# Karthik-Ragunath/RAD-NeRF

Measured on AMD Instinct MI355X. Metric: rendered frames/sec @512x512, higher is better.
Workload: dtype f32; 1 GPU; config[1]: inference 512x512, L=16 hash grid T=2^19 F=2 (xyz; ambient/torso grids tiled T=2^16 as shipped), max 16 steps/ray, 25 FPS pose stream, torso pass on; grid=hash19, engine=fused, frames_per_gpu=2122, table_dtype=f32, audio_batch=8, frames_in_flight=1, loop_launch=split, parallelism=frame-parallel x1

## Files before the change

include/radnerf_fused.h:

```cpp
#ifndef RADNERF_FUSED_H
#define RADNERF_FUSED_H

#include "radnerf_hip.h"

#ifdef __cplusplus
extern "C" {
#endif

typedef struct {
    const void *embeddings;
    const int32_t *offsets;
    uint32_t D, L, H;
    float S;
    uint32_t gridtype;
    int dtype;
} rn_grid_t;

typedef struct {
    const float *amb_w0, *amb_w1, *amb_w2;
    const float *sig_w0, *sig_w1, *sig_w2;
    const float *col_w0, *col_w1;
    uint32_t audio_dim, has_eye, ind_dim;
} rn_nerf_weights_t;

size_t rn_nerf_packed_floats(void);
size_t rn_nerf_packed_floats_h16(void);
int rn_nerf_pack_weights_h16(const rn_nerf_weights_t *w, float *packed, rn_stream_t stream);
#define RN_F32_SPLIT 2
size_t rn_nerf_packed_floats_split(void);
int rn_nerf_pack_weights_split(const rn_nerf_weights_t *w, float *packed, rn_stream_t stream);
size_t rn_nerf_bias_floats(void);
int rn_nerf_pack_weights(const rn_nerf_weights_t *w, float *packed, rn_stream_t stream);
int rn_nerf_frame_bias(const rn_nerf_weights_t *w, const float *enc_a, const float *eye, const float *ind_code,
                       float *bias, rn_stream_t stream);
int rn_nerf_frame_bias_batch(const rn_nerf_weights_t *w, const float *enc_a, uint32_t n, const float *eye, const float *ind_code,
                             float *bias, rn_stream_t stream);

int rn_nerf_fused_forward(const float *xyzs, const float *dirs, const float *deltas, uint32_t M,
                          const int32_t *m_dev, const rn_grid_t *grid_xyz, const rn_grid_t *grid_amb,
                          const float *packed, const float *bias, float bound, float *sigmas, float *rgbs,
                          float *ambient, int mlp_dtype, rn_stream_t stream);

#define RN_HEAD_STATE_INTS 64

typedef struct {
    const float *rays_o, *rays_d;
    uint32_t N;
    const float *aabb;
    float min_near;
    const uint8_t *bitfield;
    float bound, dt_gamma;
    uint32_t max_steps, cascade, grid_size;
    float T_thresh;
    float *nears, *fars;
    float *weights_sum, *depth, *image;
    int32_t *rays_alive_a, *rays_alive_b;
    float *rays_t;
    float *xyzs, *dirs, *deltas;
    float *sigmas, *rgbs;
    int32_t *state;
    uint32_t *block_counts;
    int32_t *live_slots;
    uint32_t order_w;
    const int32_t *occ_box;
} rn_head_t;

int rn_head_begin(const rn_head_t *h, rn_stream_t stream);
int rn_head_iterate(const rn_head_t *h, const rn_grid_t *grid_xyz, const rn_grid_t *grid_amb, const float *packed,
                    const float *bias, uint32_t first_iter, uint32_t n_iters, int mlp_dtype, rn_stream_t stream);
#define RN_LOOP_FIRST_MARCHED 1u
#define RN_LOOP_CLOSE_FRAME 2u
#define RN_LOOP_COOP 4u
int rn_head_iterate_ex(const rn_head_t *h, const rn_grid_t *grid_xyz, const rn_grid_t *grid_amb, const float *packed,
                       const float *bias, uint32_t first_iter, uint32_t n_iters, int mlp_dtype, uint32_t flags,
                       rn_stream_t stream);
int rn_frame_begin(const rn_head_t *h, const float *pose, float fx, float fy, float cx, float cy, uint32_t W,
                   rn_stream_t stream);
int rn_head_reschedule(const rn_head_t *h, uint32_t iter_done, uint32_t schedule_N, const int32_t *alive_total,
                       rn_stream_t stream);
#define RN_HEAD_ST_ACTIVE 4
#define RN_HEAD_ST_ITERS 16
#define RN_HEAD_ST_LIVE 17
#define RN_HEAD_ST_SLOTS 18
#define RN_HEAD_ST_UNFINISHED 19
#define RN_HEAD_ST_BARRIER 20
#define RN_HEAD_ST_STALLED 22
#define RN_HEAD_ST_HIST 32
int rn_head_check_done(const rn_head_t *h, uint32_t iters_done, rn_stream_t stream);

typedef struct {
    const float *def_w0, *def_w1, *def_w2;
    const float *tor_w0, *tor_w1, *tor_w2;
    uint32_t ind_dim;
} rn_torso_weights_t;
// ... 150 lines not shown
```

rad-nerf_amd/csrc/rn_grid.hip:

```cpp
#include "rn_scatter_dev.h"

#include <math.h>
#include <stdlib.h>

#ifndef RN_GRID_PAIR_HASHED
#define RN_GRID_PAIR_HASHED 1
#endif

namespace rn {

template <typename T, uint32_t D, uint32_t C, bool DYDX>
__device__ __forceinline__ void encode_one(const T *__restrict__ table, uint32_t off, const float (&in)[D], float scale,
                                           uint32_t resolution, uint32_t hashmap_size, uint32_t gridtype, bool align_corners,
                                           uint32_t interp, T (&results)[C], T (&grads)[DYDX ? D * C : 1]) {
    if constexpr (D == 2 || D == 3) {
        if (!align_corners && interp == 0) {
            const LevelPlan lp = plan_level<D>(scale, resolution, off, hashmap_size, gridtype, (uint32_t)(sizeof(T) * C));
            LevelFetch<T, D, C> f;
            issue_planned<T, D, C, RN_GRID_PAIR_HASHED != 0, true>(table, lp, in, f);
            blend_level<T, D, C, DYDX>(f, scale, results, grads);
            return;
        }
    }
    encode_level<T, D, C, DYDX>(table, off, in, scale, resolution, hashmap_size, gridtype, align_corners, interp, results, grads);
// ... 736 lines not shown
    if constexpr (C <= 2 && D <= 3)
        hipLaunchKernelGGL((k_grid_bwd_table_merge<T, D, C, LAYOUT>), grid, block, 0, a.stream, grad, a.inputs, a.offsets, gt, a.B, a.L,
                           a.lc, a.gridtype, a.align_corners, a.interp);
    else
        hipLaunchKernelGGL((k_grid_bwd_table<T, D, C, N_C, LAYOUT>), grid, block, 0, a.stream, grad, a.inputs, a.offsets, gt, a.B, a.L,
                           a.lc, a.gridtype, a.align_corners, a.interp);
    if (a.dy_dx && a.grad_inputs)
        hipLaunchKernelGGL((k_grid_bwd_input<T, D, C, LAYOUT>), dim3(div_up(a.B * D, 256)), block, 0, a.stream, grad,
                           static_cast<const T *>(a.dy_dx), static_cast<T *>(a.grad_inputs), a.B, a.L);
}
template <typename T, uint32_t D, uint32_t C>
static void launch_bwd(const BwdArgs &a) {
    if (a.layout == RN_LAYOUT_LBC) launch_bwd_layout<T, D, C, RN_LAYOUT_LBC>(a);
    else launch_bwd_layout<T, D, C, RN_LAYOUT_BLC>(a);
}
template <typename T, uint32_t D>
static int dispatch_bwd_c(uint32_t C, const BwdArgs &a) {
    switch (C) {
        case 1: launch_bwd<T, D, 1>(a); return RN_OK;
        case 2: launch_bwd<T, D, 2>(a); return RN_OK;
        case 4: launch_bwd<T, D, 4>(a); return RN_OK;
        case 8: launch_bwd<T, D, 8>(a); return RN_OK;
    }
    set_error("GridEncoding: C must be 1, 2, 4, or 8.");
    return RN_ERR_INVALID_ARG;
}
template <typename T>
static int dispatch_bwd_d(uint32_t D, uint32_t C, const BwdArgs &a) {
    switch (D) {
        case 2: return dispatch_bwd_c<T, 2>(C, a);
        case 3: return dispatch_bwd_c<T, 3>(C, a);
        case 4: return dispatch_bwd_c<T, 4>(C, a);
        case 5: return dispatch_bwd_c<T, 5>(C, a);
    }
    set_error("GridEncoding: D must be 2, 3, 4 or 5.");
    return RN_ERR_INVALID_ARG;
}

template <uint32_t D>
static int dispatch_tv_c(uint32_t C, const float *inputs, const float *table, float *grad, const int32_t *offsets,
                         float weight, uint32_t B, uint32_t L, const LevelConsts &lc, uint32_t gridtype, bool ac,
                         hipStream_t s) {
    const dim3 block(256), grid(div_up(B, 256), L);
    switch (C) {
        case 1: hipLaunchKernelGGL((k_grad_tv<D, 1>), grid, block, 0, s, inputs, table, grad, offsets, weight, B, lc, gridtype, ac); return RN_OK;
        case 2: hipLaunchKernelGGL((k_grad_tv<D, 2>), grid, block, 0, s, inputs, table, grad, offsets, weight, B, lc, gridtype, ac); return RN_OK;
        case 4: hipLaunchKernelGGL((k_grad_tv<D, 4>), grid, block, 0, s, inputs, table, grad, offsets, weight, B, lc, gridtype, ac); return RN_OK;
        case 8: hipLaunchKernelGGL((k_grad_tv<D, 8>), grid, block, 0, s, inputs, table, grad, offsets, weight, B, lc, gridtype, ac); return RN_OK;
    }
    set_error("GridEncoding: C must be 1, 2, 4, or 8.");
    return RN_ERR_INVALID_ARG;
}

}

using namespace rn;

extern "C" {

int rn_grid_encode_forward(const float *inputs, const void *embeddings, const int32_t *offsets, void *outputs,
                           uint32_t B, uint32_t D, uint32_t C, uint32_t L, float S, uint32_t H, void *dy_dx,
                           uint32_t gridtype, int align_corners, uint32_t interp, int dtype, int layout,
                           rn_stream_t stream) {
    if (B == 0) return RN_OK;
    RN_REQUIRE(inputs && embeddings && offsets && outputs, "grid_encode_forward: null pointer");
    RN_REQUIRE(L >= 1 && L <= kMaxLevels, "grid_encode_forward: L=%u out of range (1..%u)", L, kMaxLevels);
    RN_REQUIRE(dtype == RN_F32 || dtype == RN_F16, "grid_encode_forward: dtype must be RN_F32 or RN_F16");
    RN_REQUIRE(layout == RN_LAYOUT_LBC || layout == RN_LAYOUT_BLC || layout == RN_LAYOUT_BLC_LEVELMAJOR,
               "grid_encode_forward: bad layout");
    RN_REQUIRE(gridtype <= 1 && interp <= 1, "grid_encode_forward: bad gridtype / interpolation id");
    FwdArgs a{inputs, embeddings, offsets, outputs, B, L, make_level_consts(L, S, H), dy_dx, gridtype,
              align_corners != 0, interp, layout, as_stream(stream)};
    const int rc = (dtype == RN_F32) ? dispatch_fwd_d<float>(D, C, a) : dispatch_fwd_d<__half>(D, C, a);
    if (rc != RN_OK) return rc;
    return check_launch("grid_encode_forward");
}

size_t rn_grid_encode_forward_workspace(uint32_t B, uint32_t L, uint32_t C, int dtype) {
    const size_t per_sample = (size_t)L * C * (dtype == RN_F16 ? 2 : 4);
    const size_t chunk = B < planned_chunk_default() ? B : planned_chunk_default();
    return chunk * per_sample;
}

static int grid_forward_ws(const float *inputs, const void *embeddings, const int32_t *offsets, const int32_t *offsets_host,
                           void *outputs, uint32_t B, uint32_t D, uint32_t C, uint32_t L, float S, uint32_t H, void *dy_dx,
                           uint32_t gridtype, int align_corners, uint32_t interp, int dtype, int layout, void *workspace,
                           size_t workspace_bytes, const InXform &xf, rn_stream_t stream, const char *who) {
    if (B == 0) return RN_OK;
    RN_REQUIRE(inputs && embeddings && offsets && outputs, "%s: null pointer", who);
    RN_REQUIRE(L >= 1 && L <= kMaxLevels, "%s: L=%u out of range (1..%u)", who, L, kMaxLevels);
    RN_REQUIRE(dtype == RN_F32 || dtype == RN_F16, "%s: dtype must be RN_F32 or RN_F16", who);
    RN_REQUIRE(layout == RN_LAYOUT_LBC || layout == RN_LAYOUT_BLC, "%s: layout must be RN_LAYOUT_LBC or RN_LAYOUT_BLC", who);
    const bool shape_ok = offsets_host && !dy_dx && !align_corners && interp == 0 && (D == 2 || D == 3) && (C == 2 || C == 4) &&
                          ((uintptr_t)embeddings & 15u) == 0 && ((uintptr_t)outputs & 15u) == 0 &&
                          (layout == RN_LAYOUT_LBC || (workspace && ((uintptr_t)workspace & 15u) == 0));
    if (shape_ok) {
        PlannedArgs a{inputs, embeddings, offsets, offsets_host, outputs, B, L, make_level_consts(L, S, H), gridtype, layout, workspace,
                      workspace_bytes, as_stream(stream), xf};
        const int rc = (dtype == RN_F32) ? dispatch_planned<float>(D, C, a) : dispatch_planned<__half>(D, C, a);
        if (rc <= 0) return rc != RN_OK ? rc : check_launch(who);
    }
    RN_REQUIRE(!xf.on, "%s: only the planned shapes (offsets_host given, D in {2,3}, C in {2,4}, 16-byte aligned buffers); normalise the "
               "coordinates yourself and call rn_grid_encode_forward_ws", who);
    return rn_grid_encode_forward(inputs, embeddings, offsets, outputs, B, D, C, L, S, H, dy_dx, gridtype, align_corners, interp, dtype,
                                  layout, stream);
}

int rn_grid_encode_forward_ws(const float *inputs, const void *embeddings, const int32_t *offsets, const int32_t *offsets_host,
                              void *outputs, uint32_t B, uint32_t D, uint32_t C, uint32_t L, float S, uint32_t H, void *dy_dx,
                              uint32_t gridtype, int align_corners, uint32_t interp, int dtype, int layout, void *workspace,
                              size_t workspace_bytes, rn_stream_t stream) {
// ... 55 lines not shown
```

rad-nerf_amd/radnerf/fused.py:

```python
import ctypes as C

import numpy as np
import torch

import radnerf_hip as hip
from radnerf_hip.abi import (RN_F16, RN_F32, RN_F32_SPLIT, RN_HEAD_ST_HIST, RN_HEAD_ST_ITERS, RN_HEAD_ST_SLOTS, RN_HEAD_ST_STALLED,
                             RN_HEAD_ST_UNFINISHED, RN_HEAD_STATE_INTS, RN_LOOP_CLOSE_FRAME, RN_LOOP_COOP, RN_LOOP_FIRST_MARCHED,
                             RN_TORSO_PLAN_MAX_BYTES, GridT, HeadT, NerfWeightsT, TorsoWeightsT)

from . import switches

_lib = hip._lib


def _grid_desc(enc, table):
    g = GridT()
    g.embeddings, g.offsets = table.data_ptr(), enc.offsets.data_ptr()
    g.D, g.L, g.H = enc.input_dim, enc.num_levels, enc.base_resolution
    g.S = float(np.log2(enc.per_level_scale))
    g.gridtype = enc.gridtype_id
    g.dtype = RN_F16 if table.dtype == torch.float16 else RN_F32
    return g


def head_weights(model):
    return [l.weight for l in model.ambient_net.net] + [l.weight for l in model.sigma_net.net] + [l.weight for l in model.color_net.net]


def weights_desc(ws, audio_dim, has_eye, ind_dim):
    nw = NerfWeightsT()
    (nw.amb_w0, nw.amb_w1, nw.amb_w2, nw.sig_w0, nw.sig_w1, nw.sig_w2, nw.col_w0, nw.col_w1) = [w.data_ptr() for w in ws]
    nw.audio_dim, nw.has_eye, nw.ind_dim = audio_dim, has_eye, ind_dim
    return nw


def torso_weights(model):
    return [l.weight for l in model.torso_deform_net.net] + [l.weight for l in model.torso_net.net]


def torso_weights_desc(ws, ind_dim):
    assert tuple(ws[0].shape) == (64, 96 + ind_dim) and tuple(ws[3].shape) == (32, 128 + ind_dim)
    tw = TorsoWeightsT()
    (tw.def_w0, tw.def_w1, tw.def_w2, tw.tor_w0, tw.tor_w1, tw.tor_w2) = [w.data_ptr() for w in ws]
    tw.ind_dim = ind_dim
    return tw


def torso_constants(poses, ind_code):
    return (poses.detach().reshape(-1).contiguous().float(),
            ind_code.detach().reshape(-1).contiguous().float() if ind_code is not None else None)


def supported(model):
    try:
        ok = (model.encoder.num_levels == 16 and model.encoder.level_dim == 2 and model.encoder.input_dim == 3
              and model.encoder_ambient.num_levels == 16 and model.encoder_ambient.level_dim == 2
              and model.encoder_ambient.input_dim == 2 and model.hidden_dim == 64 and model.geo_feat_dim == 64
              and model.hidden_dim_ambient == 64 and model.hidden_dim_color == 64 and model.num_layers == 3
              and model.num_layers_ambient == 3 and model.num_layers_color == 2 and model.ambient_dim == 2
              and model.encoder_dir.degree == 4 and not model.encoder.align_corners and model.encoder.interp_id == 0)
        if model.torso:
            ok = ok and (model.torso_encoder.num_levels == 16 and model.torso_encoder.level_dim == 2
                         and model.torso_deform_net.dim_hidden == 64 and model.torso_net.dim_hidden == 32
                         and model.torso_deform_in_dim == 42 and model.pose_in_dim == 54)
        return bool(ok)
    except AttributeError:
        return False


class TorsoPlan:

    def __init__(self, key, refs, buf, n_on, stream):
        self.key, self.refs, self.buf, self.n_on, self.stream = key, refs, buf, n_on, stream
        self.event = torch.cuda.Event()
        self.event.record()
        self.waited = {stream}


class FusedState:

    def __init__(self, model):
        if not supported(model):
            raise RuntimeError("fused engine: unsupported network shape; use engine='ops'")
        self.model = model
        self.dev = model.density_bitfield.device
        n_packed = max(int(_lib.rn_nerf_packed_floats()), int(_lib.rn_nerf_packed_floats_h16()),
                       int(_lib.rn_nerf_packed_floats_split()))
        self.packed = torch.empty(n_packed, dtype=torch.float32, device=self.dev)
        self.mlp_dtype = RN_F32
        self.loop_hint = None
        self.bias = torch.empty(int(_lib.rn_nerf_bias_floats()), dtype=torch.float32, device=self.dev)
        self.tpacked = (torch.empty(int(_lib.rn_torso_packed_floats()), dtype=torch.float32, device=self.dev)
                        if model.torso else None)
        self._versions = None
        self._N = 0
        self._zero_eye = torch.zeros(1, dtype=torch.float32, device=self.dev)
        self.plan = None
        self.plan_builds = 0
        self.box = None
        self._box_key = None
        self.box_builds = 0

    def occ_box(self):
        if not switches.on("RN_OCC_BOX"):
            return None
        m = self.model
        bits = m.density_bitfield
        key = (bits.data_ptr(), bits._version, int(m.cascade), int(m.grid_size))
        if key != self._box_key:
            if self.box is None:
                self.box = torch.zeros(8, dtype=torch.int32, device=self.dev)
            hip.call("rn_occ_box", hip.ptr(bits), int(m.cascade), int(m.grid_size), hip.ptr(self.box), hip.stream())
            self._box_key = key
            self.box_builds += 1
        return self.box

    def _weights(self):
        m = self.model
        ws = head_weights(m)
        if m.torso:
            ws += torso_weights(m)
        return ws

    def refresh(self):
        ws = self._weights()
        tables = [self.model.encoder.embeddings, self.model.encoder_ambient.embeddings]
        if self.model.torso:
            tables.append(self.model.torso_encoder.embeddings)
        mlp = {"f32": RN_F32, "f16": RN_F16, "f32x2": RN_F32_SPLIT}[
            getattr(getattr(self.model, "opt", None), "mlp_dtype", "f32")]
        half = bool(getattr(getattr(self.model, "opt", None), "half_tables", False))
        versions = tuple((w._version, w.data_ptr()) for w in ws + tables) + (mlp, half)
        if versions == self._versions:
            return
        m = self.model
        for w in ws:
            if w.dtype != torch.float32 or not w.is_contiguous():
                raise RuntimeError("fused engine: MLP weights must be contiguous float32")
        self.nw = weights_desc(ws[:8], m.audio_dim, int(m.exp_eye), m.individual_dim)
        assert tuple(ws[0].shape) == (64, 32 + m.audio_dim) and tuple(ws[3].shape) == (64, 64 + int(m.exp_eye))
        assert tuple(ws[5].shape) == (65, 64) and tuple(ws[6].shape) == (64, 80 + m.individual_dim)
        self.mlp_dtype = mlp
        packer = {RN_F32: "rn_nerf_pack_weights", RN_F16: "rn_nerf_pack_weights_h16",
                  RN_F32_SPLIT: "rn_nerf_pack_weights_split"}[mlp]
        hip.call(packer, C.byref(self.nw), hip.ptr(self.packed), hip.stream())
        if m.torso:
            self.tw = torso_weights_desc(ws[8:14], m.individual_dim_torso)
            hip.call("rn_torso_pack_weights", C.byref(self.tw), hip.ptr(self.tpacked), hip.stream())
        if half:
            encs = [m.encoder, m.encoder_ambient] + ([m.torso_encoder] if m.torso else [])
            self.tables = [hip.aligned(e.half_table()) for e in encs]
        else:
            self.tables = [hip.aligned(t.detach()) for t in tables]
        self.gx = _grid_desc(m.encoder, self.tables[0])
# ... 237 lines not shown
        alpha_out = torch.empty(N, 1, dtype=torch.float32, device=dev)
    hip.call("rn_torso_fused", hip.ptr(bg_coords), N, hip.ptr(model.density_grid_torso), int(model.grid_size), float(thresh),
             hip.ptr(poses6), hip.ptr(ict), float(model.opt.torso_shrink), C.byref(st.tw), hip.ptr(st.tpacked), C.byref(st.gt),
             hip.ptr(bg_in), hip.ptr(bg_out), hip.ptr(alpha_out), hip.ptr(deform_out), hip.stream())
    return bg_out, alpha_out


def frame_bias_batch(model, codes, eye, ind_code):
    st = _state(model)
    st.refresh()
    return _frame_bias(st, codes, eye, ind_code, batch=True)


def render_frame(model, rays_o, rays_d, enc_a, ind_code, eye, bg_coords, poses, ind_code_torso, bg_color, dt_gamma,
                 max_steps, T_thresh, want_u8=False, ray_source=None, frame_bias=None):
    st = _state(model)
    st.refresh()
    N = rays_o.shape[0]
    st.scratch(N)
    dev = rays_o.device
    s = hip.stream()

    if frame_bias is None:
        bias = _frame_bias(st, enc_a, eye, ind_code)
    else:
        bias = frame_bias.reshape(-1)
        assert bias.numel() == st.bias.numel() and bias.is_contiguous() and bias.dtype == torch.float32

    weights_sum = torch.empty(N, dtype=torch.float32, device=dev)
    depth = torch.empty(N, dtype=torch.float32, device=dev)
    image = torch.empty(N, 3, dtype=torch.float32, device=dev)

    h = HeadT()
    h.rays_o, h.rays_d, h.N = rays_o.data_ptr(), rays_d.data_ptr(), N
    h.aabb, h.min_near = model.aabb_infer.data_ptr(), float(model.min_near)
    h.bitfield, h.bound, h.dt_gamma = model.density_bitfield.data_ptr(), float(model.bound), float(dt_gamma)
    h.max_steps, h.cascade, h.grid_size, h.T_thresh = int(max_steps), int(model.cascade), int(model.grid_size), float(T_thresh)
    h.nears, h.fars = st.nears.data_ptr(), st.fars.data_ptr()
    h.weights_sum, h.depth, h.image = weights_sum.data_ptr(), depth.data_ptr(), image.data_ptr()
    h.rays_alive_a, h.rays_alive_b = st.rays_alive[0].data_ptr(), st.rays_alive[1].data_ptr()
    h.rays_t = st.rays_t.data_ptr()
    h.xyzs = st.samples.data_ptr()
    h.dirs = st.samples.data_ptr() + N * 3 * 4
    h.deltas = st.samples.data_ptr() + N * 6 * 4
    h.sigmas, h.rgbs = st.sigmas.data_ptr(), st.rgbs.data_ptr()
    h.state, h.block_counts = st.state.data_ptr(), st.block_counts.data_ptr()
    h.live_slots = st.live_slots.data_ptr() if (getattr(model.opt, "live_list", True) and switches.on("RN_LIVE_LIST")) else None
    h.order_w = int(getattr(model, "ray_order_width", 0) or 0)
    h.occ_box = hip.ptr(st.occ_box())

    shard = getattr(model, "shard_schedule", None)
    merged = shard is None and getattr(model.opt, "frame_kernels", "merged") == "merged"
    n_iters = int(max_steps) if st.loop_hint is None else min(int(max_steps), st.loop_hint)
    if merged:
        if ray_source is not None:
            pose, (fx, fy, cx, cy), W = ray_source
            pose = pose.reshape(-1, 4)[:4].contiguous().float()
            hip.call("rn_frame_begin", C.byref(h), hip.ptr(pose), float(fx), float(fy), float(cx), float(cy), int(W), s)
        else:
            hip.call("rn_frame_begin", C.byref(h), None, 0.0, 0.0, 0.0, 0.0, 0, s)
        hip.call("rn_head_iterate_ex", C.byref(h), C.byref(st.gx), C.byref(st.gw), hip.ptr(st.packed), hip.ptr(bias), 0, n_iters,
                 st.mlp_dtype, RN_LOOP_FIRST_MARCHED | RN_LOOP_CLOSE_FRAME | loop_flags(model), s)
    else:
        if ray_source is not None:
            pose, (fx, fy, cx, cy), W = ray_source
            pose = pose.reshape(-1, 4)[:4].contiguous().float()
            hip.call("rn_get_rays", hip.ptr(pose), float(fx), float(fy), float(cx), float(cy), N // int(W), int(W), hip.ptr(rays_o),
                     hip.ptr(rays_d), s)
        hip.call("rn_head_begin", C.byref(h), s)
        if shard is None:
            hip.call("rn_head_iterate_ex", C.byref(h), C.byref(st.gx), C.byref(st.gw), hip.ptr(st.packed), hip.ptr(bias), 0,
                     n_iters, st.mlp_dtype, loop_flags(model), s)
        else:
            group, n_total = shard
            total = torch.empty(1, dtype=torch.int32, device=dev)
            for it in range(n_iters):
                hip.call("rn_head_iterate_ex", C.byref(h), C.byref(st.gx), C.byref(st.gw), hip.ptr(st.packed), hip.ptr(bias),
                         it, 1, st.mlp_dtype, loop_flags(model), s)
                bank = ((it + 1) & 1) * 8
                total.copy_(st.state[bank:bank + 1])
                group.all_reduce(total)
                hip.call("rn_head_reschedule", C.byref(h), it, int(n_total), hip.ptr(total), hip.stream())
        if n_iters < int(max_steps):
            hip.call("rn_head_check_done", C.byref(h), n_iters, s)

    bg_in = None
    if torch.is_tensor(bg_color):
        bg_in = bg_color.reshape(-1, 3).contiguous().float()
        if bg_in.shape[0] != N:
            bg_in = bg_in.expand(N, 3).contiguous()
    elif bg_color is not None and float(bg_color) != 1.0:
        bg_in = torch.full((N, 3), float(bg_color), dtype=torch.float32, device=dev)
    results = {}
    model.last_stats = LoopStats(st)
    u8 = torch.empty(N, 3, dtype=torch.uint8, device=dev) if want_u8 else None
    if model.torso and merged:
        thresh = min(model.density_thresh_torso, model.mean_density_torso)
        keep = getattr(model.opt, "keep_torso_layer", True)
        talpha = torch.empty(N, 1, dtype=torch.float32, device=dev) if keep else None
        bg_final = torch.empty(N, 3, dtype=torch.float32, device=dev) if keep else None
        coords = bg_coords.contiguous().float()
        p6, ict = torso_constants(poses, ind_code_torso)
        plan = st.torso_plan(bg_coords, coords, thresh)
        if plan is not None:
            hip.call("rn_torso_blend_frame_planned", hip.ptr(plan.buf), plan.buf.numel(), N, plan.n_on, hip.ptr(p6), hip.ptr(ict),
                     float(model.opt.torso_shrink), C.byref(st.tw), hip.ptr(st.tpacked), C.byref(st.gt), hip.ptr(bg_in),
                     hip.ptr(bg_final), hip.ptr(talpha), None, hip.ptr(image), hip.ptr(weights_sum), hip.ptr(depth),
                     hip.ptr(st.nears), hip.ptr(st.fars), hip.ptr(u8), s)
        else:
            hip.call("rn_torso_blend_frame", hip.ptr(coords), N, hip.ptr(model.density_grid_torso), int(model.grid_size), float(thresh),
                     hip.ptr(p6), hip.ptr(ict), float(model.opt.torso_shrink), C.byref(st.tw), hip.ptr(st.tpacked), C.byref(st.gt),
                     hip.ptr(bg_in), hip.ptr(bg_final), hip.ptr(talpha), hip.ptr(image), hip.ptr(weights_sum), hip.ptr(depth),
                     hip.ptr(st.nears), hip.ptr(st.fars), hip.ptr(u8), s)
        if keep:
            results["torso_alpha"], results["torso_color"] = talpha, bg_final
    else:
        bg_final = bg_in
        if model.torso:
            thresh = min(model.density_thresh_torso, model.mean_density_torso)
            bg_final, talpha = torso_forward(model, bg_coords, poses, ind_code_torso, thresh, bg_in=bg_in)
            results["torso_alpha"], results["torso_color"] = talpha, bg_final
        hip.call("rn_blend_frame", hip.ptr(image), hip.ptr(weights_sum), hip.ptr(bg_final), hip.ptr(depth), hip.ptr(st.nears),
                 hip.ptr(st.fars), N, hip.ptr(u8), s)
    results.update(image=image, depth=depth, weights_sum=weights_sum, nears=st.nears, fars=st.fars)
    if want_u8:
        results["image_u8"] = u8
    return results


def get_rays(pose, intrinsics, H, W):
# ... 20 lines not shown
```

rad-nerf_amd/radnerf/switches.py:

```python
import os

TABLE = (
    ("RN_ADAM", "hip", ("hip", "torch"), "optimizer of `make_optimizer` on the GPU: `HipAdam` (one update kernel for all tensors) or torch's fused Adam"),
    ("RN_ASR", "torch", ("torch", "hip"), "`Wav2Vec2CTC` (`radnerf/asr.py`) on the GPU in fp32: the same arithmetic in plain torch, or the wav2vec2 kernels (`rn_asr_*`, opt-in: bit-reproducible and independent of the batching, but 56 ms against 44 ms for a minute of audio at the real size, DESIGN.md §3)"),
    ("RN_AUDIO_TRAIN", "hip", ("hip", "torch"), "`encode_audio` on the GPU: the audio kernels (`radnerf/audio.py`) or the `nn.Module` path"),
    ("RN_LIVE_LIST", "1", ("1", "0"), "fused inference engine: hand the loop the list of live sample slots (`0`: every launch scans all slots)"),
    ("RN_MLP_TRAIN", "hip", ("hip", "torch"), "the per-operator MLP stacks under autograd: `rn_mlp64_*` (`radnerf/mlp_train.py`) or `nn.Linear`"),
    ("RN_OCC_BOX", "1", ("1", "0"), "fused inference engine: hand the loop the box around the occupancy grid's set bits (`rn_occ_box`, built once per grid): with one cascade and a constant step a ray tests only the cells between its entry into and its exit from that box (same bits); `0`: every ray tests every cell from `near` to `far`"),
    ("RN_PERCEP", "hip", ("hip", "torch"), "`PerceptualAlex` (`radnerf/percep.py`) on the GPU in fp32: the perceptual kernels (`rn_percep_*`), or the same arithmetic in plain torch (unfold + matmul)"),
    ("RN_SCATTER", "lbc", ("lbc", "binned"), "table-gradient scatter: the line merge for every level, or hashed levels of the first grid summed by table region"),
    ("RN_TORSO_PLAN", "1", ("1", "0"), "fused inference engine: a frame whose pixel grid and torso occupancy grid are those of the frame before runs its torso pass over a plan built once (`rn_torso_plan_build`: the covered pixels and their position encoding; same bits); `0`: every frame computes them (`rn_torso_blend_frame`)"),
    ("RN_TORSO_STEP", "device", ("device", "host"), "with `RN_TORSO_TRAIN=fused`: the whole torso step on a device-side count, or the fused layer on the index list the host asks for"),
    ("RN_TORSO_TRAIN", "ops", ("ops", "fused"), "torso layer of a training call: the per-operator layers, or the fused kernels of `radnerf/train_torso.py` (opt-in)"),
    ("RN_TRAIN_CAMERA", "torch", ("torch", "fused"), "pose code of `--train_camera`: torch's expressions, or `rn_camera_rays_*` (`radnerf/train_camera.py`, opt-in; lets a captured camera step keep the fused head)"),
    ("RN_TRAIN_DETERMINISTIC", "0", ("0", "1"), "`1`: a step on the fused routes (head, `RN_TRAIN_CAMERA=fused`, `RN_TORSO_TRAIN=fused`) runs no float atomic, eager or captured: the table gradients are summed in one fixed order (`rn_grid_scatter_ordered`; takes precedence over `RN_SCATTER`) and the audio nets' parameter gradients through per-workgroup partials -- two runs from the same seeds give the same bits (opt-in: slower)"),
    ("RN_TRAIN_GLUE", "hip", ("hip", "torch"), "elementwise glue of the per-operator step: single kernels (`radnerf/train_glue.py`) or the PyTorch expressions"),
    ("RN_TRAIN_HEAD", "fused", ("fused", "ops"), "`NeRFNetwork.forward` of a training call: one forward and one backward kernel (`radnerf/train_head.py`) or the per-operator path"),
    ("RN_TRAIN_HEAD_ZERO", "0", ("0", "1"), "`1`: the fused head zero-fills its output rows past the live count (for tools that look at all rows)"),
    ("RN_TRAIN_LOSS", "fused", ("fused", "torch"), "head loss of `train_step`: blend, clamp and loss in one kernel, or the PyTorch expression"),
    ("RN_TRAIN_MARCH", "step", ("step", "ops"), "marcher of a budgeted step: one launch with near / far and the counters, or `near_far_from_aabb` + `rn_march_rays_train_budget`"),
    ("RN_TRAIN_MLP", "f32", ("f32", "f16"), "matrix products of the fused head (`RN_TRAIN_HEAD=fused`): fp32 matrix cores, or 16-bit operands with fp32 sums (`rn_train_head_*_h16`, opt-in: the arithmetic of the reference's `-O` runs for its `nn.Linear` layers; saved tiles, tables and gradients stay fp32)"),
    ("RN_TRAIN_NOISE", "hash", ("hash", "torch"), "jitter of the one-launch marcher: the launch's own hash, or `torch.rand` as the reference draws it (the test suite pins this)"),
    ("RN_TRAIN_OVERLAP", "1", ("1", "0"), "table-gradient scatter and audio nets on side streams beside the step (`0`: everything on one stream)"),
    ("RN_TRAIN_PACKED", "1", ("1", "0"), "`SyntheticTrainStream.batch`: one gather kernel into one flat buffer (`0`: separate tensors, as a generic loader hands over)"),
    ("RN_TRAIN_SET", "hip", ("hip", "torch"), "`DeviceTrainSet.batch` on the GPU: one launch, or the plain-torch restatement of `collate`"),
)
_ROWS = {row[0]: row for row in TABLE}


def get(name):
    _, default, accepted, _ = _ROWS[name]
    value = os.environ.get(name, default)
    if value not in accepted:
        raise ValueError(f"{name}={value!r} is not one of its accepted values: {' | '.join(accepted)}")
    return value


def on(name):
    return get(name) == "1"


def markdown():
    rows = ["| switch | default | accepted | selects |", "|---|---|---|---|"]
    rows += ["| `%s` | `%s` | %s | %s |" % (name, default, " \\| ".join("`%s`" % v for v in accepted), doc) for name, default, accepted, doc in TABLE]
    return "\n".join(rows)


if __name__ == "__main__":
    print(markdown())
```

rad-nerf_amd/radnerf_hip/abi.py:

```python
import ctypes as C

_int, _u32, _f32, _f64, _sz, _ptr, _P = C.c_int, C.c_uint32, C.c_float, C.c_double, C.c_size_t, C.c_void_p, C.POINTER
_i64 = C.c_int64

RN_F32, RN_F16 = 0, 1
RN_LAYOUT_LBC, RN_LAYOUT_BLC, RN_LAYOUT_BLC_LEVELMAJOR = 0, 1, 2

RN_F32_SPLIT = 2
RN_HEAD_STATE_INTS = 64
RN_TORSO_PLAN_MAX_BYTES = 256 << 20
RN_LOOP_FIRST_MARCHED, RN_LOOP_CLOSE_FRAME, RN_LOOP_COOP = 1, 2, 4
RN_HEAD_ST_ACTIVE, RN_HEAD_ST_ITERS, RN_HEAD_ST_LIVE, RN_HEAD_ST_SLOTS = 4, 16, 17, 18
RN_HEAD_ST_UNFINISHED, RN_HEAD_ST_STALLED, RN_HEAD_ST_HIST = 19, 22, 32


class GridT(C.Structure):
    c_name = "rn_grid_t"
    _fields_ = [("embeddings", _ptr), ("offsets", _ptr), ("D", _u32), ("L", _u32), ("H", _u32), ("S", _f32),
                ("gridtype", _u32), ("dtype", _int)]


class NerfWeightsT(C.Structure):
    c_name = "rn_nerf_weights_t"
    _fields_ = [("amb_w0", _ptr), ("amb_w1", _ptr), ("amb_w2", _ptr), ("sig_w0", _ptr), ("sig_w1", _ptr),
# ... 77 lines not shown
    "rn_device_count": (_int, []),
    "rn_prof_enable": (_int, [_int]),
    "rn_prof_pause": (_int, [_int]),
    "rn_prof_collect": (_int, [C.POINTER(_u32), C.POINTER(_f32)]),
    "rn_prof_durations": (_int, [C.POINTER(_f32), _u32]),
    "rn_near_far_from_aabb": (_int, [_ptr, _ptr, _ptr, _u32, _f32, _ptr, _ptr, _ptr]),
    "rn_sph_from_ray": (_int, [_ptr, _ptr, _f32, _u32, _ptr, _ptr]),
    "rn_morton3D": (_int, [_ptr, _u32, _ptr, _ptr]),
    "rn_morton3D_invert": (_int, [_ptr, _u32, _ptr, _ptr]),
    "rn_packbits": (_int, [_ptr, _u32, _f32, _ptr, _ptr]),
    "rn_morton3D_dilation": (_int, [_ptr, _u32, _u32, _ptr, _ptr]),
    "rn_march_rays_train_workspace": (_sz, [_u32]),
    "rn_march_rays_train": (_int, [_ptr, _ptr, _ptr, _f32, _f32, _u32, _u32, _u32, _u32, _u32, _ptr, _ptr, _ptr, _ptr, _ptr,
                                   _ptr, _ptr, _ptr, _ptr, _ptr]),
    "rn_march_rays_train_budget": (_int, [_ptr, _ptr, _ptr, _f32, _f32, _u32, _u32, _u32, _u32, _u32, _ptr, _ptr, _ptr, _ptr,
                                          _ptr, _ptr, _ptr, _ptr, _ptr, _ptr, _ptr]),
    "rn_march_rays_train_step_state": (_sz, [_u32]),
    "rn_march_rays_train_step": (_int, [_ptr, _ptr, _ptr, _ptr, _f32, _f32, _f32, _u32, _u32, _u32, _u32, _u32, _ptr, _ptr,
                                        _ptr, _ptr, _ptr, _ptr, _ptr, _ptr, _ptr, _ptr, _u32, _ptr]),
    "rn_march_rays_train_backward": (_int, [_ptr, _ptr, _ptr, _ptr, _u32, _u32, _ptr, _ptr, _ptr]),
    "rn_composite_rays_train_forward": (_int, [_ptr, _ptr, _ptr, _ptr, _ptr, _u32, _u32, _f32, _ptr, _ptr, _ptr, _ptr, _ptr]),
    "rn_composite_rays_train_backward": (_int, [_ptr, _ptr, _ptr, _ptr, _ptr, _ptr, _ptr, _ptr, _ptr, _ptr, _ptr, _u32, _u32,
                                                _f32, _ptr, _ptr, _ptr, _ptr]),
    "rn_march_rays": (_int, [_u32, _u32, _ptr, _ptr, _ptr, _ptr, _f32, _f32, _u32, _u32, _u32, _ptr, _ptr, _ptr, _ptr, _ptr,
                             _ptr, _ptr, _ptr, _ptr]),
    "rn_composite_rays": (_int, [_u32, _u32, _f32, _ptr, _ptr, _ptr, _ptr, _ptr, _ptr, _ptr, _ptr, _ptr, _ptr]),
    "rn_compact_rays_workspace": (_sz, [_u32]),
    "rn_compact_rays": (_int, [_ptr, _u32, _ptr, _ptr, _ptr, _ptr, _ptr]),
    "rn_grid_encode_forward": (_int, [_ptr, _ptr, _ptr, _ptr, _u32, _u32, _u32, _u32, _f32, _u32, _ptr, _u32, _int, _u32, _int,
                                      _int, _ptr]),
    "rn_grid_encode_forward_workspace": (_sz, [_u32, _u32, _u32, _int]),
    "rn_grid_encode_forward_ws": (_int, [_ptr, _ptr, _ptr, _ptr, _ptr, _u32, _u32, _u32, _u32, _f32, _u32, _ptr, _u32, _int,
                                         _u32, _int, _int, _ptr, _sz, _ptr]),
    "rn_grid_encode_forward_bound": (_int, [_ptr, _f32, _ptr, _ptr, _ptr, _ptr, _u32, _u32, _u32, _u32, _f32, _u32, _u32, _int,
                                            _int, _ptr, _sz, _ptr]),
    "rn_grid_encode_backward": (_int, [_ptr, _ptr, _ptr, _ptr, _ptr, _u32, _u32, _u32, _u32, _f32, _u32, _ptr, _ptr, _u32, _int,
                                       _u32, _int, _int, _ptr]),
    "rn_grad_total_variation": (_int, [_ptr, _ptr, _ptr, _ptr, _f32, _u32, _u32, _u32, _u32, _f32, _u32, _u32, _int, _ptr]),
    "rn_sh_encode_forward": (_int, [_ptr, _ptr, _u32, _u32, _u32, _ptr, _ptr]),
    "rn_sh_encode_backward": (_int, [_ptr, _ptr, _u32, _u32, _u32, _ptr, _ptr, _ptr]),
    "rn_freq_encode_forward": (_int, [_ptr, _u32, _u32, _u32, _u32, _ptr, _ptr]),
    "rn_freq_encode_backward": (_int, [_ptr, _ptr, _u32, _u32, _u32, _u32, _ptr, _ptr]),
    "rn_nerf_packed_floats": (_sz, []),
    "rn_nerf_packed_floats_h16": (_sz, []),
    "rn_nerf_pack_weights_h16": (_int, [_P(NerfWeightsT), _ptr, _ptr]),
    "rn_nerf_packed_floats_split": (_sz, []),
    "rn_nerf_pack_weights_split": (_int, [_P(NerfWeightsT), _ptr, _ptr]),
    "rn_nerf_bias_floats": (_sz, []),
    "rn_nerf_pack_weights": (_int, [_P(NerfWeightsT), _ptr, _ptr]),
    "rn_nerf_frame_bias": (_int, [_P(NerfWeightsT), _ptr, _ptr, _ptr, _ptr, _ptr]),
    "rn_nerf_frame_bias_batch": (_int, [_P(NerfWeightsT), _ptr, _u32, _ptr, _ptr, _ptr, _ptr]),
    "rn_nerf_fused_forward": (_int, [_ptr, _ptr, _ptr, _u32, _ptr, _P(GridT), _P(GridT), _ptr, _ptr, _f32, _ptr, _ptr, _ptr,
                                     _int, _ptr]),
    "rn_head_begin": (_int, [_P(HeadT), _ptr]),
    "rn_head_iterate": (_int, [_P(HeadT), _P(GridT), _P(GridT), _ptr, _ptr, _u32, _u32, _int, _ptr]),
    "rn_head_iterate_ex": (_int, [_P(HeadT), _P(GridT), _P(GridT), _ptr, _ptr, _u32, _u32, _int, _u32, _ptr]),
    "rn_frame_begin": (_int, [_P(HeadT), _ptr, _f32, _f32, _f32, _f32, _u32, _ptr]),
    "rn_head_reschedule": (_int, [_P(HeadT), _u32, _u32, _ptr, _ptr]),
    "rn_head_check_done": (_int, [_P(HeadT), _u32, _ptr]),
    "rn_torso_packed_floats": (_sz, []),
    "rn_torso_pack_weights": (_int, [_P(TorsoWeightsT), _ptr, _ptr]),
    "rn_torso_fused": (_int, [_ptr, _u32, _ptr, _u32, _f32, _ptr, _ptr, _f32, _P(TorsoWeightsT), _ptr, _P(GridT), _ptr, _ptr,
                              _ptr, _ptr, _ptr]),
    "rn_torso_blend_frame": (_int, [_ptr, _u32, _ptr, _u32, _f32, _ptr, _ptr, _f32, _P(TorsoWeightsT), _ptr, _P(GridT), _ptr,
                                    _ptr, _ptr, _ptr, _ptr, _ptr, _ptr, _ptr, _ptr, _ptr]),
    "rn_torso_plan_bytes": (_sz, [_u32, _u32]),
    "rn_torso_plan_build": (_int, [_ptr, _u32, _ptr, _u32, _f32, _f32, _ptr, _sz, C.POINTER(_u32), _ptr]),
    "rn_torso_blend_frame_planned": (_int, [_ptr, _sz, _u32, _u32, _ptr, _ptr, _f32, _P(TorsoWeightsT), _ptr, _P(GridT), _ptr, _ptr,
                                            _ptr, _ptr, _ptr, _ptr, _ptr, _ptr, _ptr, _ptr, _ptr]),
    "rn_torso_mask": (_int, [_ptr, _u32, _ptr, _u32, _f32, _ptr, _ptr]),
    "rn_blend_frame": (_int, [_ptr, _ptr, _ptr, _ptr, _ptr, _ptr, _u32, _ptr, _ptr]),
    "rn_occupancy_workspace": (_sz, [_u32, _u32]),
    "rn_occupancy_points": (_int, [_u32, _u32, _f32, _ptr, _u32, _ptr, _ptr]),
    "rn_occupancy_update": (_int, [_ptr, _f32, _ptr, _u32, _u32, _f32, _f32, _ptr, _ptr, _ptr, _ptr]),
    "rn_mark_untrained_grid": (_int, [_ptr, _u32, _u32, _f64, _f64, _f64, _f64, _u32, _u32, _f32, _ptr, _ptr]),
    "rn_torso_grid_points": (_int, [_u32, _ptr, _u32, _ptr, _ptr]),
    "rn_torso_grid_update": (_int, [_ptr, _ptr, _u32, _f32, _ptr, _ptr]),
    "rn_occ_box": (_int, [_ptr, _u32, _u32, _ptr, _ptr]),
    "rn_hash_u01_bits": (_u32, [_u32, _u32]),
    "rn_audio_encode_windows": (_int, [_P(AudioWeightsT), _ptr, _u32, _ptr, _ptr, _ptr]),
    "rn_audio_encode_windows_backward": (_int, [_P(AudioWeightsT), _ptr, _u32, _ptr, _ptr, _P(AudioGradsT), _ptr, _ptr]),
    "rn_audio_train_acts_floats": (_sz, [_u32, _int]),
    "rn_audio_encode_windows_train": (_int, [_P(AudioWeightsT), _ptr, _u32, _ptr, _ptr, _ptr, _ptr]),
    "rn_audio_encode_windows_backward_acts": (_int, [_P(AudioWeightsT), _ptr, _u32, _ptr, _ptr, _P(AudioGradsT), _ptr, _ptr,
                                                     _ptr]),
    "rn_audio_backward_partials_floats": (_sz, [_u32, _int]),
    "rn_audio_encode_windows_backward_ordered": (_int, [_P(AudioWeightsT), _ptr, _u32, _ptr, _ptr, _P(AudioGradsT), _ptr, _ptr,
                                                        _ptr, _ptr]),
    "rn_audio_encode_stream": (_int, [_P(AudioWeightsT), _ptr, _u32, _u32, _u32, _ptr, _ptr, _ptr]),
    "rn_audio_smooth": (_int, [_ptr, _u32, _u32, _f32, _ptr, _int, _ptr]),
    "rn_audio_smooth_seq": (_int, [_ptr, _u32, _u32, _f32, _ptr, _int, _ptr, _ptr]),
    "rn_get_rays": (_int, [_ptr, _f32, _f32, _f32, _f32, _u32, _u32, _ptr, _ptr, _ptr]),
    "rn_get_bg_coords": (_int, [_u32, _u32, _ptr, _ptr]),
    "rn_convert_poses": (_int, [_ptr, _u32, _ptr, _ptr]),
    "rn_mlp64_image_floats": (_sz, [_u32, _u32, _u32]),
    "rn_mlp64_tile_floats": (_sz, [_u32]),
    "rn_mlp64_wgrad_workspace": (_sz, [_u32]),
    "rn_mlp64_pack": (_int, [_ptr, _u32, _ptr, _ptr, _u32, _u32, _u32, _ptr, _ptr]),
    "rn_mlp64_forward": (_int, [_ptr, _u32, _ptr, _ptr, _u32, _u32, _u32, _ptr, _ptr, _ptr, _ptr]),
    "rn_mlp64_backward": (_int, [_ptr, _u32, _ptr, _u32, _u32, _u32, _ptr, _ptr, _ptr, _ptr, _ptr, _ptr]),
    "rn_mlp64_weight_grads": (_int, [_ptr, _ptr, _u32, _u32, _u32, _u32, _ptr, _ptr, _ptr, _ptr, _ptr, _u32, _ptr, _ptr, _ptr,
                                     _ptr, _ptr]),
    "rn_head_mid_forward": (_int, [_ptr, _ptr, _u32, _u32, _ptr, _ptr, _ptr]),
    "rn_head_mid_backward": (_int, [_ptr, _ptr, _ptr, _u32, _u32, _ptr, _ptr]),
    "rn_abs_sum2_forward": (_int, [_ptr, _u32, _ptr, _ptr]),
    "rn_abs_sum2_backward": (_int, [_ptr, _ptr, _u32, _ptr, _ptr]),
# ... 86 lines not shown
```

Baseline: 1339 frames/s.

## Read coarser hashed xyz levels from a dense lattice image built once

Adds a planner and a build kernel that re-store the coarser hashed levels of the xyz hash grid as full dense lattices, up to a memory budget (384 MiB by default). The fused inference loop then gets a grid descriptor pointing at this image with new offsets. The existing level_is_hashed check switches those levels to direct lattice indexing, so neighbouring samples fall on shared cache lines instead of scattered hash slots. The image is rebuilt only when the table pointer or version changes, and is skipped on the first frame and during graph capture. The cost is extra device memory, a one-time build, and a larger footprint for the finer densified levels, which could hurt cache hit rates.

```diff
diff --git a/include/radnerf_fused.h b/include/radnerf_fused.h
--- a/include/radnerf_fused.h
+++ b/include/radnerf_fused.h
@@ -40,6 +40,11 @@
                           const int32_t *m_dev, const rn_grid_t *grid_xyz, const rn_grid_t *grid_amb,
                           const float *packed, const float *bias, float bound, float *sigmas, float *rgbs,
                           float *ambient, int mlp_dtype, rn_stream_t stream);
+
+int rn_grid_dense_plan(const rn_grid_t *grid, const int32_t *offsets_host, size_t budget_bytes, int32_t *image_offsets,
+                       uint32_t *levels, size_t *image_bytes);
+int rn_grid_dense_build(const rn_grid_t *grid, const int32_t *offsets_host, const int32_t *image_offsets, uint32_t levels,
+                        void *image, size_t image_bytes, rn_stream_t stream);
 
 #define RN_HEAD_STATE_INTS 64
 
diff --git a/rad-nerf_amd/csrc/rn_grid.hip b/rad-nerf_amd/csrc/rn_grid.hip
--- a/rad-nerf_amd/csrc/rn_grid.hip
+++ b/rad-nerf_amd/csrc/rn_grid.hip
@@ -812,11 +812,117 @@
     return RN_ERR_INVALID_ARG;
 }
 
+template <typename ROW>
+__global__ void __launch_bounds__(256) k_grid_dense_level(const ROW *__restrict__ src, ROW *__restrict__ dst, uint32_t n_rows,
+                                                          uint32_t src_size, uint32_t resolution, uint32_t taken) {
+    const uint32_t i = blockIdx.x * 256 + threadIdx.x;
+    if (i >= n_rows) return;
+    ROW v{};
+    if (!taken) {
+        v = src[i];
+    } else {
+        const uint32_t r1 = resolution + 1, plane = r1 * r1;
+        const uint32_t z = i / plane, rem = i - z * plane, y = rem / r1;
+        if (z < r1) {
+            const uint32_t pg[3] = {rem - y * r1, y, z};
+            v = src[grid_row<3>(0u, false, src_size, resolution, pg)];
+        }
+    }
+    dst[i] = v;
+}
+
+struct DensePlan {
+    uint32_t rows[kMaxLevels];
+    uint32_t levels;
+    uint64_t total_rows;
+};
+
+static uint64_t dense_level_rows(uint32_t resolution) {
+    const uint64_t r1 = (uint64_t)resolution + 1u;
+    return (r1 * r1 * r1 + 7u) & ~(uint64_t)7u;
+}
+
+static bool dense_plan(const rn_grid_t *g, const int32_t *oh, size_t budget_bytes, DensePlan &dp) {
+    if (g->gridtype != 0 || g->D != 3) return false;
+    const LevelConsts lc = make_level_consts(g->L, g->S, g->H);
+    const uint64_t row_bytes = g->dtype == RN_F16 ? 4u : 8u;
+    dp.levels = 0;
+    dp.total_rows = 0;
+    for (uint32_t l = 0; l < g->L; l++) dp.total_rows += (dp.rows[l] = (uint32_t)(oh[l + 1] - oh[l]));
+    for (uint32_t l = 0; l < g->L; l++) {
+        if (!level_is_hashed(3, lc.resolution[l], dp.rows[l], 0u)) continue;
+        const uint64_t full = dense_level_rows(lc.resolution[l]), rows = dp.total_rows - dp.rows[l] + full;
+        if (rows * row_bytes > budget_bytes || rows * row_bytes >= (1ull << 32) || rows >= (1ull << 31)) break;
+        dp.total_rows = rows;
+        dp.rows[l] = (uint32_t)full;
+        dp.levels |= 1u << l;
+    }
+    return dp.levels != 0;
+}
+
+static int check_dense_grid(const rn_grid_t *g, const int32_t *oh, const char *who) {
+    RN_REQUIRE(g && oh, "%s: null pointer", who);
+    RN_REQUIRE(g->L >= 1 && g->L <= kMaxLevels, "%s: L=%u out of range (1..%u)", who, g->L, kMaxLevels);
+    RN_REQUIRE(g->dtype == RN_F32 || g->dtype == RN_F16, "%s: dtype must be RN_F32 or RN_F16", who);
+    for (uint32_t l = 0; l < g->L; l++) RN_REQUIRE(oh[l + 1] > oh[l] && oh[l] >= 0, "%s: offsets must ascend from >= 0", who);
+    return RN_OK;
+}
+
 }
 
 using namespace rn;
 
 extern "C" {
+
+int rn_grid_dense_plan(const rn_grid_t *grid, const int32_t *offsets_host, size_t budget_bytes, int32_t *image_offsets,
+                       uint32_t *levels, size_t *image_bytes) {
+    const int rc = check_dense_grid(grid, offsets_host, "grid_dense_plan");
+    if (rc != RN_OK) return rc;
+    RN_REQUIRE(image_offsets && levels && image_bytes, "grid_dense_plan: null pointer");
+    DensePlan dp;
+    if (!dense_plan(grid, offsets_host, budget_bytes, dp)) return 0;
+    image_offsets[0] = 0;
+    for (uint32_t l = 0; l < grid->L; l++) image_offsets[l + 1] = image_offsets[l] + (int32_t)dp.rows[l];
+    *levels = dp.levels;
+    *image_bytes = (size_t)dp.total_rows * (grid->dtype == RN_F16 ? 4u : 8u);
+    return 1;
+}
+
+int rn_grid_dense_build(const rn_grid_t *grid, const int32_t *offsets_host, const int32_t *image_offsets, uint32_t levels,
+                        void *image, size_t image_bytes, rn_stream_t stream) {
+    const int rc = check_dense_grid(grid, offsets_host, "grid_dense_build");
+    if (rc != RN_OK) return rc;
+    RN_REQUIRE(grid->embeddings && image_offsets && image, "grid_dense_build: null pointer");
+    RN_REQUIRE(grid->gridtype == 0 && grid->D == 3, "grid_dense_build: a hash grid with D = 3");
+    RN_REQUIRE(((uintptr_t)grid->embeddings & 7u) == 0 && ((uintptr_t)image & 15u) == 0, "grid_dense_build: unaligned table or image");
+    const LevelConsts lc = make_level_consts(grid->L, grid->S, grid->H);
+    const size_t row_bytes = grid->dtype == RN_F16 ? 4u : 8u;
+    uint64_t at = 0;
+    for (uint32_t l = 0; l < grid->L; l++) {
+        const uint32_t size = (uint32_t)(offsets_host[l + 1] - offsets_host[l]);
+        const bool taken = (levels >> l) & 1u;
+        RN_REQUIRE(!taken || level_is_hashed(3, lc.resolution[l], size, 0u), "grid_dense_build: level %u is not hashed", l);
+        RN_REQUIRE((uint64_t)image_offsets[l] == at, "grid_dense_build: image_offsets[%u] does not follow from the levels", l);
+        at += taken ? dense_level_rows(lc.resolution[l]) : size;
+        RN_REQUIRE(at < (1ull << 31) && at * row_bytes < (1ull << 32), "grid_dense_build: image of 4 GiB or 2^31 rows and more");
+    }
+    RN_REQUIRE((uint64_t)image_offsets[grid->L] == at && at * row_bytes == image_bytes,
+               "grid_dense_build: image_bytes does not follow from the levels");
+    for (uint32_t l = 0; l < grid->L; l++) {
+        const uint32_t size = (uint32_t)(offsets_host[l + 1] - offsets_host[l]);
+        const uint32_t n_rows = (uint32_t)(image_offsets[l + 1] - image_offsets[l]), taken = (levels >> l) & 1u;
+        const char *src = static_cast<const char *>(grid->embeddings) + (size_t)offsets_host[l] * row_bytes;
+        char *dst = static_cast<char *>(image) + (size_t)image_offsets[l] * row_bytes;
+        const dim3 blocks(div_up(n_rows, 256));
+        if (grid->dtype == RN_F16)
+            hipLaunchKernelGGL((k_grid_dense_level<uint32_t>), blocks, dim3(256), 0, as_stream(stream), reinterpret_cast<const uint32_t *>(src),
+                               reinterpret_cast<uint32_t *>(dst), n_rows, size, lc.resolution[l], taken);
+        else
+            hipLaunchKernelGGL((k_grid_dense_level<uint2>), blocks, dim3(256), 0, as_stream(stream), reinterpret_cast<const uint2 *>(src),
+                               reinterpret_cast<uint2 *>(dst), n_rows, size, lc.resolution[l], taken);
+    }
+    return check_launch("grid_dense_build");
+}
 
 int rn_grid_encode_forward(const float *inputs, const void *embeddings, const int32_t *offsets, void *outputs,
                            uint32_t B, uint32_t D, uint32_t C, uint32_t L, float S, uint32_t H, void *dy_dx,
diff --git a/rad-nerf_amd/radnerf/fused.py b/rad-nerf_amd/radnerf/fused.py
--- a/rad-nerf_amd/radnerf/fused.py
+++ b/rad-nerf_amd/radnerf/fused.py
@@ -21,6 +21,13 @@
     g.gridtype = enc.gridtype_id
     g.dtype = RN_F16 if table.dtype == torch.float16 else RN_F32
     return g
+
+
+def _image_desc(g, image, offsets):
+    d = GridT()
+    C.pointer(d)[0] = g
+    d.embeddings, d.offsets = image.data_ptr(), offsets.data_ptr()
+    return d
 
 
 def head_weights(model):
@@ -72,6 +79,15 @@
 
     def __init__(self, key, refs, buf, n_on, stream):
         self.key, self.refs, self.buf, self.n_on, self.stream = key, refs, buf, n_on, stream
+        self.event = torch.cuda.Event()
+        self.event.record()
+        self.waited = {stream}
+
+
+class DenseImage:
+
+    def __init__(self, key, table, buf, offsets, gx, levels, stream):
+        self.key, self.table, self.buf, self.offsets, self.gx, self.levels, self.stream = key, table, buf, offsets, gx, levels, stream
         self.event = torch.cuda.Event()
         self.event.record()
         self.waited = {stream}
@@ -100,6 +116,57 @@
         self.box = None
         self._box_key = None
         self.box_builds = 0
+        self.dense_builds = 0
+
+    def frame_grid(self):
+        if not switches.on("RN_DENSE_LEVELS") or torch.cuda.is_current_stream_capturing():
+            return self.gx
+        m = self.model
+        table = self.tables[0]
+        mb = getattr(getattr(m, "opt", None), "dense_budget_mb", None)
+        budget = int(switches.get("RN_DENSE_BUDGET_MB") if mb is None else mb) << 20
+        key = (table.data_ptr(), m.encoder.embeddings._version, table.dtype, budget)
+        img = getattr(m, "_fused_dense", None)
+        if img is not None and img.key != key:
+            img = None
+            object.__setattr__(m, "_fused_dense", None)
+        if img is None:
+            seen = getattr(m, "_fused_dense_seen", None)
+            object.__setattr__(m, "_fused_dense_seen", key)
+            if seen != key:
+                return self.gx
+            img = self._build_dense(key, table, budget)
+            object.__setattr__(m, "_fused_dense", img)
+        if img.buf is None:
+            return self.gx
+        cur = torch.cuda.current_stream()
+        if cur.cuda_stream not in img.waited:
+            cur.wait_event(img.event)
+            img.buf.record_stream(cur)
+            img.offsets.record_stream(cur)
+            img.waited.add(cur.cuda_stream)
+        return img.gx
+
+    def _build_dense(self, key, table, budget):
+        enc = self.model.encoder
+        oh = hip.host_offsets(enc.offsets)
+        new_off = (C.c_int32 * (enc.num_levels + 1))()
+        levels, nbytes = C.c_uint32(0), C.c_size_t(0)
+        rc = _lib.rn_grid_dense_plan(C.byref(self.gx), oh, budget, new_off, C.byref(levels), C.byref(nbytes))
+        if rc < 0:
+            raise RuntimeError(f"rn_grid_dense_plan failed ({rc}): {hip.last_error()}")
+        buf = offsets = gx = None
+        if rc == 1:
+            try:
+                buf = torch.empty(nbytes.value, dtype=torch.uint8, device=self.dev)
+                offsets = torch.tensor(list(new_off), dtype=torch.int32, device=self.dev)
+            except torch.cuda.OutOfMemoryError:
+                buf = None
+        if buf is not None:
+            hip.call("rn_grid_dense_build", C.byref(self.gx), oh, new_off, levels.value, hip.ptr(buf), nbytes.value, hip.stream())
+            gx = _image_desc(self.gx, buf, offsets)
+            self.dense_builds += 1
+        return DenseImage(key, table, buf, offsets, gx, levels.value, torch.cuda.current_stream().cuda_stream)
 
     def occ_box(self):
         if not switches.on("RN_OCC_BOX"):
@@ -443,6 +510,7 @@
     shard = getattr(model, "shard_schedule", None)
     merged = shard is None and getattr(model.opt, "frame_kernels", "merged") == "merged"
     n_iters = int(max_steps) if st.loop_hint is None else min(int(max_steps), st.loop_hint)
+    gx = st.frame_grid()
     if merged:
         if ray_source is not None:
             pose, (fx, fy, cx, cy), W = ray_source
@@ -450,7 +518,7 @@
             hip.call("rn_frame_begin", C.byref(h), hip.ptr(pose), float(fx), float(fy), float(cx), float(cy), int(W), s)
         else:
             hip.call("rn_frame_begin", C.byref(h), None, 0.0, 0.0, 0.0, 0.0, 0, s)
-        hip.call("rn_head_iterate_ex", C.byref(h), C.byref(st.gx), C.byref(st.gw), hip.ptr(st.packed), hip.ptr(bias), 0, n_iters,
+        hip.call("rn_head_iterate_ex", C.byref(h), C.byref(gx), C.byref(st.gw), hip.ptr(st.packed), hip.ptr(bias), 0, n_iters,
                  st.mlp_dtype, RN_LOOP_FIRST_MARCHED | RN_LOOP_CLOSE_FRAME | loop_flags(model), s)
     else:
         if ray_source is not None:
@@ -460,13 +528,13 @@
                      hip.ptr(rays_d), s)
         hip.call("rn_head_begin", C.byref(h), s)
         if shard is None:
-            hip.call("rn_head_iterate_ex", C.byref(h), C.byref(st.gx), C.byref(st.gw), hip.ptr(st.packed), hip.ptr(bias), 0,
+            hip.call("rn_head_iterate_ex", C.byref(h), C.byref(gx), C.byref(st.gw), hip.ptr(st.packed), hip.ptr(bias), 0,
                      n_iters, st.mlp_dtype, loop_flags(model), s)
         else:
             group, n_total = shard
             total = torch.empty(1, dtype=torch.int32, device=dev)
             for it in range(n_iters):
-                hip.call("rn_head_iterate_ex", C.byref(h), C.byref(st.gx), C.byref(st.gw), hip.ptr(st.packed), hip.ptr(bias),
+                hip.call("rn_head_iterate_ex", C.byref(h), C.byref(gx), C.byref(st.gw), hip.ptr(st.packed), hip.ptr(bias),
                          it, 1, st.mlp_dtype, loop_flags(model), s)
                 bank = ((it + 1) & 1) * 8
                 total.copy_(st.state[bank:bank + 1])
diff --git a/rad-nerf_amd/radnerf/switches.py b/rad-nerf_amd/radnerf/switches.py
--- a/rad-nerf_amd/radnerf/switches.py
+++ b/rad-nerf_amd/radnerf/switches.py
@@ -4,6 +4,8 @@
     ("RN_ADAM", "hip", ("hip", "torch"), "optimizer of `make_optimizer` on the GPU: `HipAdam` (one update kernel for all tensors) or torch's fused Adam"),
     ("RN_ASR", "torch", ("torch", "hip"), "`Wav2Vec2CTC` (`radnerf/asr.py`) on the GPU in fp32: the same arithmetic in plain torch, or the wav2vec2 kernels (`rn_asr_*`, opt-in: bit-reproducible and independent of the batching, but 56 ms against 44 ms for a minute of audio at the real size, DESIGN.md §3)"),
     ("RN_AUDIO_TRAIN", "hip", ("hip", "torch"), "`encode_audio` on the GPU: the audio kernels (`radnerf/audio.py`) or the `nn.Module` path"),
+    ("RN_DENSE_BUDGET_MB", "384", ("160", "384", "896", "2304"), "with `RN_DENSE_LEVELS=1`: the most memory, in MiB, the dense image of the xyz table may take (`opt.dense_budget_mb`, any number, overrides it); for the T = 2^19 hash grid in fp32 the four values store levels 5-8 (149 MiB), 5-9 (343 MiB), 5-10 (857 MiB) and 5-11 (2215 MiB) as lattices, fp16 tables take half"),
+    ("RN_DENSE_LEVELS", "1", ("1", "0"), "fused inference engine: a frame whose xyz table is that of the frame before reads the coarser hashed levels from a dense image built once (`rn_grid_dense_build`: each such level stored as its whole lattice, so neighbouring samples share cache lines; same features, same bits); `0`: every frame gathers from the hashed table"),
     ("RN_LIVE_LIST", "1", ("1", "0"), "fused inference engine: hand the loop the list of live sample slots (`0`: every launch scans all slots)"),
     ("RN_MLP_TRAIN", "hip", ("hip", "torch"), "the per-operator MLP stacks under autograd: `rn_mlp64_*` (`radnerf/mlp_train.py`) or `nn.Linear`"),
     ("RN_OCC_BOX", "1", ("1", "0"), "fused inference engine: hand the loop the box around the occupancy grid's set bits (`rn_occ_box`, built once per grid): with one cascade and a constant step a ray tests only the cells between its entry into and its exit from that box (same bits); `0`: every ray tests every cell from `near` to `far`"),
diff --git a/rad-nerf_amd/radnerf_hip/abi.py b/rad-nerf_amd/radnerf_hip/abi.py
--- a/rad-nerf_amd/radnerf_hip/abi.py
+++ b/rad-nerf_amd/radnerf_hip/abi.py
@@ -153,6 +153,8 @@
     "rn_nerf_frame_bias_batch": (_int, [_P(NerfWeightsT), _ptr, _u32, _ptr, _ptr, _ptr, _ptr]),
     "rn_nerf_fused_forward": (_int, [_ptr, _ptr, _ptr, _u32, _ptr, _P(GridT), _P(GridT), _ptr, _ptr, _f32, _ptr, _ptr, _ptr,
                                      _int, _ptr]),
+    "rn_grid_dense_plan": (_int, [_P(GridT), _ptr, _sz, _ptr, _P(_u32), _P(_sz)]),
+    "rn_grid_dense_build": (_int, [_P(GridT), _ptr, _ptr, _u32, _ptr, _sz, _ptr]),
     "rn_head_begin": (_int, [_P(HeadT), _ptr]),
     "rn_head_iterate": (_int, [_P(HeadT), _P(GridT), _P(GridT), _ptr, _ptr, _u32, _u32, _int, _ptr]),
     "rn_head_iterate_ex": (_int, [_P(HeadT), _P(GridT), _P(GridT), _ptr, _ptr, _u32, _u32, _int, _u32, _ptr]),
```

Result: faster. 1352 frames/s (median of 6 runs) (+1.0%).
